# ActiveVisionLab/CrossScore

Measured on AMD Instinct MI355X. Metric: query-images/sec at 518x518, 5 ref views, bs=8; score-map MAE vs ref, higher is better.
Workload: dtype fp16

## Files before the change

crossscore_amd/_lib.py:

```python
from __future__ import annotations

import ctypes as C
import os

HERE = os.path.dirname(os.path.abspath(__file__))
LIB_PATH = os.path.join(HERE, "libcrossscore_hip.so")

CS_OK, CS_ERR_BAD_ARG, CS_ERR_UNSUPPORTED, CS_ERR_STATE, CS_ERR_HIP = range(5)
METRIC_SSIM_M1_1, METRIC_SSIM_0_1, METRIC_MAE, METRIC_MSE = range(4)
PNG_GRAY16, PNG_RGB8 = 0, 1
PNG_DYNAMIC, PNG_ADAPTIVE_FILTER = 1, 2
(PNGDEC_OK, PNGDEC_BAD_CRC, PNGDEC_BAD_ADLER, PNGDEC_BAD_ZLIB_HEADER, PNGDEC_BAD_BLOCK_TYPE, PNGDEC_BAD_STORED_LEN, PNGDEC_BAD_CODE, PNGDEC_BAD_SYMBOL,
 PNGDEC_BAD_DISTANCE, PNGDEC_STREAM_SHORT, PNGDEC_STREAM_LONG, PNGDEC_BAD_FILTER, PNGDEC_INPUT_EXHAUSTED, PNGDEC_HEADER_MISMATCH,
 PNGDEC_BAD_FRAMING) = range(15)
JPEG_GRAY, JPEG_444, JPEG_422, JPEG_420 = range(4)
(JPGDEC_OK, JPGDEC_BAD_FRAMING, JPGDEC_HEADER_MISMATCH, JPGDEC_BAD_TABLE, JPGDEC_BAD_CODE, JPGDEC_BAD_SYMBOL, JPGDEC_INPUT_EXHAUSTED,
 JPGDEC_BAD_RESTART) = range(8)
JPGDEC_BAD_SCAN = 8
JPEG_PROGRESSIVE = 1
GTMAP_SSIM, GTMAP_MAE = 0, 1

DTYPE_F32, DTYPE_F16, DTYPE_BF16 = 0, 1, 2
(EPI_BIAS_F16, EPI_BIAS_GELU_F16, EPI_BIAS_RELU_F16, EPI_BIAS_LEAKY_F16, EPI_RESID_F32, EPI_PATCH_F32, EPI_HEAD_SCORE,
 EPI_LN_F16, EPI_LN_GELU_F16, EPI_RESID_F32_LN) = range(10)
# ... 41 lines not shown
    "cs_finalize": (_i, [_vp]),
    "cs_forward": (_i, [_vp, _vp, _vp, _i, _i, _i, _i, _vp, _vp, _i, _vp, _vp]),
    "cs_encode_references": (_i, [_vp, _vp, _i, _i, _i, _vp, _vp]),
    "cs_forward_cached": (_i, [_vp, _vp, _vp, _i, _i, _i, _i, _vp, _vp, _i, _vp, _vp]),
    "cs_forward_u8": (_i, [_vp, _vp, _vp, _i, _i, _i, _i, _fp, _fp, _vp, _vp, _i, _vp, _vp]),
    "cs_encode_references_u8": (_i, [_vp, _vp, _i, _i, _i, _fp, _fp, _vp, _vp]),
    "cs_forward_cached_u8": (_i, [_vp, _vp, _vp, _i, _i, _i, _i, _fp, _fp, _vp, _vp, _i, _vp, _vp]),
    "cs_u8_input_supported": (_i, [_vp, _vp, _i, _i]),
    "cs_op_token_descriptors": (_i, [_vp, _i, _i, _i, _i, _vp, _vp]),
    "cs_op_descriptor_centre": (_i, [_vp, _i, _i, _vp, _vp]),
    "cs_op_descriptor_unit": (_i, [_vp, _i, _i, _vp, _vp, _vp]),
    "cs_op_select_references": (_i, [_vp, _i, _vp, _i, _i, _vp, _i, _vp, _vp, _vp]),
    "cs_op_gather_tokens": (_i, [_vp, _i, _i, _i, _vp, _i, _i, _vp, _vp]),
    "cs_forward_select": (_i, [_vp, _vp, _vp, _vp, _vp, _i, _vp, _i, _i, _i, _i, _vp, _vp, _i, _vp, _vp, _vp, _vp]),
    "cs_forward_select_u8": (_i, [_vp, _vp, _vp, _vp, _vp, _i, _vp, _i, _i, _i, _i, _fp, _fp, _vp, _vp, _i, _vp, _vp, _vp, _vp]),
    "cs_op_group_descriptors": (_i, [_vp, _i, _i, _vp, _i, _vp, _vp, _vp]),
    "cs_op_select_references_grouped": (_i, [_vp, _i, _vp, _vp, _vp, _vp, _i, _i, _i, _vp, _i, _vp, _vp, _vp]),
    "cs_op_gather_tokens_ex": (_i, [_vp, _i, _i, _i, _vp, _i, _i, _vp, _vp, _i]),
    "cs_forward_select_grouped": (_i, [_vp, _vp, _vp, _vp, _vp, _i, _vp, _i, _vp, _i, _vp, _i, _i, _i, _i, _vp, _vp, _i, _vp, _vp, _vp, _vp]),
    "cs_forward_select_grouped_u8": (_i, [_vp, _vp, _vp, _vp, _vp, _i, _vp, _i, _vp, _i, _vp, _i, _i, _i, _i, _fp, _fp, _vp, _vp, _i, _vp, _vp,
                                          _vp, _vp]),
    "cs_workspace_bytes": (_sz, [_vp, _i, _i, _i, _i]),
    "cs_nonfinite_count": (_i, [_vp, C.POINTER(C.c_longlong)]),
    "cs_forward_stats": (_i, [_vp, C.POINTER(C.c_int), C.POINTER(C.c_double), C.c_char_p, _sz]),
    "cs_debug_set_op_operand_dtype": (_i, [_i]),
    "cs_debug_capture": (_i, [_vp, _i]),
    "cs_debug_read": (_i, [_vp, C.c_char_p, _vp, _sz, C.POINTER(C.c_int), C.POINTER(C.c_int), C.POINTER(C.c_int64), _vp]),
    "cs_profile_enable": (_i, [_vp, _i]),
    "cs_profile_read": (_i, [_vp, _i, C.POINTER(C.c_double), C.POINTER(C.c_int), C.POINTER(C.c_double)]),
    "cs_profile_read_bytes": (_i, [_vp, _i, C.POINTER(C.c_double)]),
    "cs_op_gemm": (_i, [_vp, _i, _vp, _i, _i, _i, _i, _vp, _vp, _i, _vp, _i, _i, _vp, _i, _i, _i, _i, _f,
                        _vp, _vp, _i, _vp, _i, _vp, _f, _vp]),
    "cs_op_head_score": (_i, [_vp, _i, _vp, _i, _i, _i, _vp, _vp, _i, _i, _i, _i, _f, _vp, _vp, _vp, _vp]),
    "cs_op_attention": (_i, [_vp, _vp, _vp, _vp, _i, _i, _i, _i, _ll, _ll, _ll, _ll, _i, _i, _i, _i, _i, _f, _vp, _vp]),
    "cs_op_attention_weights": (_i, [_vp, _vp, _i, _i, _ll, _ll, _i, _i, _i, _i, _i, _f, _vp, _i, _vp, _vp]),
    "cs_op_reference_use": (_i, [_vp, _vp, _i, _i, _ll, _ll, _i, _i, _i, _i, _i, _i, _f, _vp, _vp, _vp, _vp, _vp, _vp]),
    "cs_request_reference_use": (_i, [_vp, _vp, _vp, _vp, _vp]),
    "cs_op_layernorm": (_i, [_vp, _i, _i, _vp, _vp, _f, _vp, _vp, _vp]),
    "cs_op_ln_finalize": (_i, [_vp, _i, _i, _i, _i, _f, _vp, _vp]),
    "cs_op_silu_mul": (_i, [_vp, _i, _i, _i, _vp]),
    "cs_op_im2col": (_i, [_vp, _vp, _i, _i, _i, _i, _i, _vp]),
    "cs_op_patch_embed": (_i, [_vp, _vp, _vp, _vp, _i, _i, _i, _i, _i, _i, _vp, _vp]),
    "cs_op_patch_embed_fused": (_i, [_vp, _vp, _vp, _vp, _i, _i, _i, _i, _i, _vp, _vp]),
    "cs_op_patch_embed_fused_u8": (_i, [_vp, _i, _i, _i, _i, _i, _i, _i, _i, _i, _i, _fp, _fp, _vp, _vp, _vp, _i, _i, _vp, _vp]),
    "cs_debug_patch_fused_enable": (None, [_i]),
    "cs_set_lanes": (_i, [_vp, _i]),
    "cs_redraw_lane_streams": (_i, [_vp]),
    "cs_debug_stream_probe_log": (None, [_i]),
    "cs_op_pos_bicubic": (_i, [_vp, _i, _i, _i, _i, _vp, _vp]),
    "cs_op_pos_bicubic_ex": (_i, [_vp, _i, _i, _i, _i, _i, _vp, _vp]),
    "cs_op_pe_bilinear": (_i, [_vp, _i, _i, _i, _i, _i, _vp, _vp]),
    "cs_op_pe_interp": (_i, [_vp, _i, _i, _i, _i, _i, _i, _vp, _vp]),
    "cs_op_score_to_gray16": (_i, [_vp, C.c_longlong, _i, _vp, _vp]),
    "cs_op_score_to_rgb": (_i, [_vp, C.c_longlong, C.c_float, C.c_float, _vp, _vp, _vp]),
    "cs_png_bound": (_sz, [_i, _i, _i]),
    "cs_png_workspace_bytes": (_sz, [_i, _i, _i, _i]),
    "cs_op_png_encode": (_i, [_vp, _i, _i, _i, _i, _ll, _vp, _sz, _vp, _vp, _vp]),
    "cs_op_png_encode_ex": (_i, [_vp, _i, _i, _i, _i, _ll, _vp, _sz, _vp, _vp, _vp, _i]),
    "cs_png_probe": (_i, [_vp, _sz, _vp, _vp, _i]),
    "cs_png_decode_workspace_bytes": (_sz, [_i, _i, _i, _i, _sz]),
    "cs_op_png_decode": (_i, [_vp, _vp, _vp, _vp, _vp, _sz, _i, _i, _i, _i, _vp, _ll, _vp, _vp, _vp]),
    "cs_jpeg_probe": (_i, [_vp, _sz, _vp]),
    "cs_jpeg_decode_workspace_bytes": (_sz, [_i, _i, _i, _sz]),
    "cs_op_jpeg_decode": (_i, [_vp, _vp, _vp, _sz, _i, _i, _i, _vp, _ll, _vp, _vp, _vp]),
    "cs_jpeg_probe_ex": (_i, [_vp, _sz, _i, _vp, _vp]),
    "cs_jpeg_decode_workspace_bytes_ex": (_sz, [_i, _i, _i, _sz, _i]),
    "cs_op_jpeg_decode_ex": (_i, [_vp, _vp, _vp, _sz, _i, _i, _i, _vp, _ll, _vp, _vp, _i, _vp]),
    "cs_debug_jpeg_scan_levels": (None, [_i]),
    "cs_op_denorm_to_rgb8": (_i, [_vp, _i, _i, _i, _fp, _fp, _vp, _vp]),
    "cs_op_metric_map_u16": (_i, [_vp, _i, _i, _i, _i, _i, _i, _i, _i, _i, _i, _i, _vp, _vp, _vp]),
    "cs_op_gt_metric_map_u8": (_i, [_vp, _vp, _i, _i, _i, _ll, _i, _vp, _i, _vp]),
    "cs_op_metric_map_sums_u16": (_i, [_vp, _vp, _i, _i, _i, _i, _ll, _vp, _vp]),
    "cs_op_gt_metric_sums_u8": (_i, [_vp, _vp, _i, _i, _i, _ll, _vp, _vp]),
    "cs_score_gt_workspace_bytes": (_sz, [_i, _i, _i]),
    "cs_op_score_gt_stats": (_i, [_vp, _vp, _i, _i, _i, _vp, _vp, _vp]),
    "cs_op_preprocess_u8": (_i, [_vp, _i, _i, _i, _i, _i, _i, _i, _i, _i, C.POINTER(C.c_float), C.POINTER(C.c_float), _vp, _vp, _vp]),
    "cs_op_pack_f16": (_i, [_vp, _i, _i, _vp, _i, _vp, _vp, _vp]),
    "cs_op_streams_overlap": (_i, [_vp, _vp, _vp]),
    "cs_op_ln_fold_consts": (_i, [_vp, _i, _vp, _vp, _vp, _i, _i, _vp, _vp, _vp]),
    "cs_gemm_column_tiles": (_i, [_i]),
    "cs_debug_gemm256_enable": (None, [_i]),
    "cs_debug_gemm256_kmin": (None, [_i]),
    "cs_debug_gemm_grid": (None, [_i]),
    "cs_debug_panel_impl": (None, [_i]),
    "cs_panel_supported": (_i, [_i, _i]),
    "cs_panel_image_bytes": (_sz, [_i]),
    "cs_op_panel_pack": (_i, [_vp, _vp, _vp, _vp, _vp, _vp, _vp, _vp]),
    "cs_op_linear_layernorm": (_i, [_vp, _vp, _vp, _vp, _vp, _vp, _f, _vp, _vp, _i, _i, _vp]),
    "cs_op_linear_layernorm_linear": (_i, [_vp, _vp, _vp, _vp, _vp, _vp, _f, _vp, _vp, _vp, _vp, _i, _i, _vp, _i, _i, _vp]),
    "cs_debug_rowln_enable": (None, [_i]),
    "cs_op_encoder_panel": (_i, [_vp, _vp, _vp, _vp, _vp, _vp, _vp, _i, _f, _vp]),
}

_lib = None


class CrossScoreHipError(RuntimeError):
    pass


def load() -> C.CDLL:
    global _lib
    if _lib is not None:
        return _lib
    if not os.path.exists(LIB_PATH):
        raise CrossScoreHipError(
            f"{LIB_PATH} is missing: build it with `python -m crossscore_amd.build` (hipcc --offload-arch=gfx950). "
            "The CrossScore hot path has no CPU/eager fallback.")
    lib = C.CDLL(LIB_PATH)
    for name, (res, args) in SYMBOLS.items():
        fn = getattr(lib, name)
        fn.restype = res
        fn.argtypes = args
    _lib = lib
    return lib


def last_error() -> str:
    return load().cs_last_error().decode("utf-8", "replace")


def check(rc: int) -> None:
    if rc == CS_OK:
        return
    msg = last_error()
    if rc in (CS_ERR_BAD_ARG,):
        raise ValueError(msg)
    if rc == CS_ERR_UNSUPPORTED:
        raise NotImplementedError(msg)
    raise CrossScoreHipError(msg)
```

crossscore_amd/csrc/attention.hip:

```cpp
#include "cs_common.h"
#include <atomic>
#include <math.h>
#include <type_traits>

#ifdef CS_ATTN_STAMP
__device__ unsigned long long g_attn_dbg[64 * 4 * 8];
#define CS_TS(k) do { __builtin_amdgcn_sched_barrier(0); const unsigned long long now_ = __builtin_amdgcn_s_memtime(); \
    ph[k] += now_ - tlast; tlast = now_; __builtin_amdgcn_sched_barrier(0); } while (0)
#else
#define CS_TS(k) do { } while (0)
#endif

namespace {

template <int DH>
struct AttnCfg {
  static constexpr bool T16 = DH == 48 || DH == 64;
  static constexpr int KS = DH / 16;
  static constexpr int DT = (DH + 31) / 32;
  static constexpr int KS2 = (DH + 31) / 32;
  static constexpr int DT16 = DH / 16;
  static constexpr int CH = DH / 8;
  static constexpr int KROW = T16 ? 160 : DH * 2 + 16;
  static constexpr int VROW = T16 ? (DH == 64 ? 160 : 96) : (DH <= 16) ? 64 : (DH <= 96 ? 192 : (DH <= 128 ? 320 : 448));
  static_assert(T16 ? (VROW >= DH * 2 && (VROW / 4) % 16 == 8 && KROW >= KS2 * 64 && (KROW / 16) % 4 == 2)
                    : (VROW >= DT * 64 && (VROW / 4) % 32 == 16), "K / V row pitch");
  static constexpr int KTILE = 64 * KROW;
  static constexpr int VTILE = 64 * VROW;
  static constexpr int STAGE = KTILE + VTILE;
  static constexpr int NIT = (64 * CH + 255) / 256;
};

template <int DH, bool BF>
__global__ __launch_bounds__(256, DH > 128 ? 1 : (AttnCfg<DH>::T16 ? 3 : 2)) void cs_attn_kernel(CsAttnParams p) {
  using Cfg = AttnCfg<DH>;
  constexpr int KS = Cfg::KS, DT = Cfg::DT, CH = Cfg::CH, NIT = Cfg::NIT;
  extern __shared__ __attribute__((aligned(16))) char smem[];
  const int tid = threadIdx.x;
  const int lane = tid & 63;
  const int wv = __builtin_amdgcn_readfirstlane(tid >> 6);
  const int r = lane & 31;
  const int hh = lane >> 5;
  const int QB = (p.Lq + 127) / 128;
  const int xcd = blockIdx.x & 7, jj = blockIdx.x >> 3;
  const int gi = jj / QB, qb = jj - gi * QB;
  const int grp = gi * 8 + xcd;
  if (grp >= p.heads * p.nbatch) return;
  const int head = grp % p.heads;
  const int bat = grp / p.heads;
  const int q0 = qb * 128 + wv * 32;

  const h16_t* Qb = p.Q + (size_t)bat * p.q_bs + head * DH;
  const h16_t* Kb = p.K + (size_t)bat * p.k_bs + head * DH;
  const h16_t* Vb = p.V + (size_t)bat * p.v_bs + head * DH;

  constexpr bool kFullLast = (64 * CH) % 256 == 0;
  int skey[NIT], sch[NIT];
#pragma unroll
  for (int it = 0; it < NIT; ++it) {
    const int c = tid + it * 256;
    skey[it] = c / CH;
    sch[it] = c - skey[it] * CH;
  }
  uint4 kreg[NIT], vreg[NIT];
#pragma unroll
  for (int it = 0; it < NIT; ++it) { kreg[it] = make_uint4(0, 0, 0, 0); vreg[it] = make_uint4(0, 0, 0, 0); }
  unsigned kgo[NIT], vgo[NIT];
#pragma unroll
  for (int it = 0; it < NIT; ++it) {
    kgo[it] = ((unsigned)skey[it] * (unsigned)p.ldk + (unsigned)sch[it] * 8u) * 2u;
    vgo[it] = ((unsigned)skey[it] * (unsigned)p.ldv + (unsigned)sch[it] * 8u) * 2u;
  }
  const unsigned k_bytes = (unsigned)(((size_t)(p.Lk - 1) * p.ldk + DH) * 2), v_bytes = (unsigned)(((size_t)(p.Lk - 1) * p.ldv + DH) * 2);
#define CS_ATTN_LOAD_TILE(T)                                                                       \
  {                                                                                                \
    const unsigned ks_ = (unsigned)(T) * 64u * (unsigned)p.ldk * 2u, vs_ = (unsigned)(T) * 64u * (unsigned)p.ldv * 2u; \
    const __amdgpu_buffer_rsrc_t k_rs = __builtin_amdgcn_make_buffer_rsrc(                         \
        const_cast<char*>(reinterpret_cast<const char*>(Kb)) + ks_, 0, (int)(k_bytes - ks_), 0x00020000); \
    const __amdgpu_buffer_rsrc_t v_rs = __builtin_amdgcn_make_buffer_rsrc(                         \
        const_cast<char*>(reinterpret_cast<const char*>(Vb)) + vs_, 0, (int)(v_bytes - vs_), 0x00020000); \
    _Pragma("unroll") for (int it = 0; it < NIT; ++it) {                                           \
      if (kFullLast || it + 1 < NIT || tid + it * 256 < 64 * CH) {                                 \
        kreg[it] = __builtin_bit_cast(uint4, __builtin_amdgcn_raw_buffer_load_b128(k_rs, kgo[it], 0, 0)); \
        vreg[it] = __builtin_bit_cast(uint4, __builtin_amdgcn_raw_buffer_load_b128(v_rs, vgo[it], 0, 0)); \
      }                                                                                            \
    }                                                                                              \
  }
#define CS_ATTN_WRITE_TILE(BUF)                                                                    \
  _Pragma("unroll") for (int it = 0; it < NIT; ++it) {                                             \
    if (kFullLast || it + 1 < NIT || tid + it * 256 < 64 * CH) {                                   \
      char* kb_ = smem + (BUF) * Cfg::STAGE;                                                       \
      *reinterpret_cast<uint4*>(kb_ + skey[it] * Cfg::KROW + sch[it] * 16) = kreg[it];             \
      *reinterpret_cast<uint4*>(kb_ + Cfg::KTILE + skey[it] * Cfg::VROW + sch[it] * 16) = vreg[it]; \
    }                                                                                              \
  }

  if constexpr (Cfg::T16) {
    constexpr int KS2 = Cfg::KS2, DT16 = Cfg::DT16;
    const int li = lane & 15, g = lane >> 4;
    const int nqt = __builtin_amdgcn_readfirstlane(q0 >= p.Lq ? 0 : (q0 + 16 >= p.Lq ? 1 : 2));
    if constexpr (DH == 48) {
      const int zrow = (tid >> 1) & 63;
      *reinterpret_cast<uint4*>(smem + (tid >> 7) * Cfg::STAGE + zrow * Cfg::KROW + 96 + 16 * (tid & 1)) = make_uint4(0, 0, 0, 0);
    }
    h16x8_t qf[2][KS2];
#pragma unroll
    for (int qt = 0; qt < 2; ++qt) {
      int qr = q0 + 16 * qt + li;
      qr = qr < p.Lq ? qr : p.Lq - 1;
      const h16_t* qp = Qb + (size_t)qr * p.ldq + 8 * g;
#pragma unroll
      for (int s = 0; s < KS2; ++s) {
#pragma unroll
        for (int j = 0; j < 8; ++j) qf[qt][s][j] = (_Float16)0.f;
        if (32 * s + 32 <= DH || 32 * s + 8 * g < DH) qf[qt][s] = *reinterpret_cast<const h16x8_t*>(qp + 32 * s);
      }
    }
    {
      const float sc = p.scale_log2e;
      if (sc != 1.0f) {
#pragma unroll
        for (int qt = 0; qt < 2; ++qt)
#pragma unroll
          for (int s = 0; s < KS2; ++s)
#pragma unroll
            for (int j = 0; j < 8; ++j) {
              const _Float16 e = qf[qt][s][j];
              qf[qt][s][j] = __builtin_bit_cast(_Float16, f2o<BF>(o2f<BF>(__builtin_bit_cast(h16_t, e)) * sc));
            }
      }
    }
    f32x4_t ot[2][DT16];
#pragma unroll
    for (int qt = 0; qt < 2; ++qt)
#pragma unroll
      for (int d = 0; d < DT16; ++d)
#pragma unroll
        for (int e = 0; e < 4; ++e) ot[qt][d][e] = 0.f;
    constexpr float kTau = 8.0f;
    float m_run[2] = {0.f, 0.f};
    float l_run[2] = {0.f, 0.f};
    f32x4_t negm[2];
#pragma unroll
    for (int qt = 0; qt < 2; ++qt)
#pragma unroll
      for (int e = 0; e < 4; ++e) negm[qt][e] = 0.f;

    const int koff = li * Cfg::KROW + g * 16;
    const int voff = (4 * g + (li >> 2)) * Cfg::VROW + (li & 3) * 8;

    const int nt = (p.Lk + 63) / 64;
    CS_ATTN_LOAD_TILE(0)
    CS_ATTN_WRITE_TILE(0)
    __syncthreads();
#ifdef CS_ATTN_STAMP
    unsigned long long ph[5] = {0, 0, 0, 0, 0};
    const unsigned long long tbegin = __builtin_amdgcn_s_memtime(), rbegin = __builtin_amdgcn_s_memrealtime();
    unsigned long long tlast = tbegin;
#endif
    auto tile = [&](auto full_c, const int t, const int nkt) __attribute__((always_inline)) {
      constexpr bool FULL = decltype(full_c)::value;
      const char* kb = smem + (t & 1) * Cfg::STAGE;
      const char* vb = kb + Cfg::KTILE;
      f32x4_t st[2][4];
      h16x8_t pf[2][2];
      float tm[2] = {-INFINITY, -INFINITY};
#pragma unroll
      for (int kt = 0; kt < 4; ++kt) {
        if (FULL || kt < nkt) {
          if (!FULL) __builtin_amdgcn_sched_barrier(0);
#pragma unroll
          for (int s = 0; s < KS2; ++s) {
            const h16x8_t kf = *reinterpret_cast<const h16x8_t*>(kb + koff + kt * 16 * Cfg::KROW + s * 64);
#pragma unroll
            for (int qt = 0; qt < 2; ++qt)
              if (FULL || qt < nqt) st[qt][kt] = mfma_16x16x32<BF>(kf, qf[qt][s], s == 0 ? negm[qt] : st[qt][kt]);
          }
#pragma unroll
          for (int qt = 0; qt < 2; ++qt)
            if (FULL || qt < nqt) {
              if (!FULL) {
                const int key = t * 64 + kt * 16 + 4 * g;
#pragma unroll
                for (int j = 0; j < 4; ++j)
                  if (key + j >= p.Lk) st[qt][kt][j] = -INFINITY;
              }
#pragma unroll
              for (int j = 0; j < 4; ++j) tm[qt] = fmaxf(tm[qt], st[qt][kt][j]);
            }
        }
      }
      CS_TS(0);
      if (t == 0 || __builtin_amdgcn_ballot_w64(fmaxf(tm[0], tm[1]) > kTau) != 0) {
#pragma unroll
        for (int qt = 0; qt < 2; ++qt)
          if (FULL || qt < nqt) {
            float rm = fmaxf(tm[qt], __shfl_xor(tm[qt], 16, 64));
            rm = fmaxf(rm, __shfl_xor(rm, 32, 64));
            const float delta = t == 0 ? rm : fmaxf(rm, 0.f);
            const float alpha = t == 0 ? 1.0f : __builtin_amdgcn_exp2f(-delta);
            m_run[qt] += delta;
#pragma unroll
            for (int e = 0; e < 4; ++e) negm[qt][e] = -m_run[qt];
            asm volatile("" : "+v"(negm[qt]));
#pragma unroll
            for (int kt = 0; kt < 4; ++kt)
              if (FULL || kt < nkt)
#pragma unroll
                for (int j = 0; j < 4; ++j) st[qt][kt][j] -= delta;
            l_run[qt] *= alpha;
#pragma unroll
            for (int d = 0; d < DT16; ++d)
#pragma unroll
              for (int e = 0; e < 4; ++e) ot[qt][d][e] *= alpha;
          }
      }
      if (!FULL) __builtin_amdgcn_sched_barrier(0);
#pragma unroll
      for (int qt = 0; qt < 2; ++qt)
        if (FULL || qt < nqt) {
          float ps0 = 0.f, ps1 = 0.f;
#pragma unroll
          for (int kt = 0; kt < 4; ++kt) {
            if (FULL || kt < nkt) {
#pragma unroll
              for (int j = 0; j < 4; j += 2) {
                const float pa = __builtin_amdgcn_exp2f(st[qt][kt][j]);
                const float pb = __builtin_amdgcn_exp2f(st[qt][kt][j + 1]);
                ps0 += pa;
                ps1 += pb;
                pf[qt][kt >> 1][4 * (kt & 1) + j] = __builtin_bit_cast(_Float16, f2o<BF>(pa));
                pf[qt][kt >> 1][4 * (kt & 1) + j + 1] = __builtin_bit_cast(_Float16, f2o<BF>(pb));
              }
            } else {
#pragma unroll
              for (int j = 0; j < 4; ++j) pf[qt][kt >> 1][4 * (kt & 1) + j] = (_Float16)0.f;
            }
          }
          l_run[qt] += ps0 + ps1;
        }
      CS_TS(1);
      if (!FULL) __builtin_amdgcn_sched_barrier(0);
#pragma unroll
      for (int s = 0; s < 2; ++s)
        if (FULL || 2 * s < nkt) {
          const char* vrow = vb + voff + 32 * s * Cfg::VROW;
#pragma unroll
          for (int d = 0; d < DT16; ++d) {
            short4_t lo = __builtin_amdgcn_ds_read_tr16_b64_v4i16(
                (__attribute__((address_space(3))) short4_t*)(vrow + d * 32));
            short4_t hi = __builtin_amdgcn_ds_read_tr16_b64_v4i16(
                (__attribute__((address_space(3))) short4_t*)(vrow + 16 * Cfg::VROW + d * 32));
            const short8_t vf8 = __builtin_shufflevector(lo, hi, 0, 1, 2, 3, 4, 5, 6, 7);
#pragma unroll
            for (int qt = 0; qt < 2; ++qt)
              if (FULL || qt < nqt) ot[qt][d] = mfma_16x16x32<BF>(__builtin_bit_cast(h16x8_t, vf8), pf[qt][s], ot[qt][d]);
          }
        }
      CS_TS(2);
    };
    auto run = [&](auto full_c, const int t0, const int t1) __attribute__((always_inline)) {
      for (int t = t0; t < t1; ++t) {
        if (t + 1 < nt) { CS_ATTN_LOAD_TILE(t + 1) }
        if (decltype(full_c)::value || nqt > 0) {
          const int left = p.Lk - t * 64;
          tile(full_c, t, left >= 64 ? 4 : (left + 15) >> 4);
        }
        if (t + 1 < nt) { CS_ATTN_WRITE_TILE((t + 1) & 1) }
        CS_TS(3);
        __syncthreads();
        CS_TS(4);
      }
    };
    const int ntf = nqt == 2 ? ((p.Lk & 63) ? nt - 1 : nt) : 0;
    run(std::true_type{}, 0, ntf);
    run(std::false_type{}, ntf, nt);
#ifdef CS_ATTN_STAMP
    if (blockIdx.x % 50 == 0 && blockIdx.x / 50 < 64 && lane == 0) {
      unsigned long long* d = g_attn_dbg + (blockIdx.x / 50 * 4 + wv) * 8;
      for (int k = 0; k < 5; ++k) d[k] = ph[k];
      d[5] = rbegin;
      d[6] = __builtin_amdgcn_s_memtime() - tbegin;
      d[7] = __builtin_amdgcn_s_memrealtime() - rbegin;
    }
#endif

    const int le = __builtin_amdgcn_mbcnt_hi(~0u, __builtin_amdgcn_mbcnt_lo(~0u, 0u));
    const int lie = le & 15, ge = le >> 4;
#pragma unroll
    for (int qt = 0; qt < 2; ++qt) {
      float l_tot = l_run[qt] + __shfl_xor(l_run[qt], 16, 64);
      l_tot += __shfl_xor(l_tot, 32, 64);
      const float inv = 1.0f / l_tot;
      const int q = q0 + 16 * qt + lie;
      if (q < p.Lq) {
        h16_t* op = p.O + (size_t)bat * p.o_bs + (size_t)q * p.ldo + head * DH + 4 * ge;
#pragma unroll
        for (int d = 0; d < DT16; ++d) {
          uint2 o;
          o.x = pack_o16x2<BF>(ot[qt][d][0] * inv, ot[qt][d][1] * inv);
          o.y = pack_o16x2<BF>(ot[qt][d][2] * inv, ot[qt][d][3] * inv);
          *reinterpret_cast<uint2*>(op + 16 * d) = o;
        }
        if (p.lse && ge == 0) p.lse[((size_t)bat * p.heads + head) * p.Lq + q] = m_run[qt] + log2f(l_tot);
      }
    }
  } else
  {
  h16x8_t qf[KS];
  {
    int qr = q0 + r;
    qr = qr < p.Lq ? qr : p.Lq - 1;
    const h16_t* qp = Qb + (size_t)qr * p.ldq + 8 * hh;
#pragma unroll
    for (int s = 0; s < KS; ++s) qf[s] = *reinterpret_cast<const h16x8_t*>(qp + 16 * s);
  }

  f32x16_t ot[DT];
#pragma unroll
  for (int d = 0; d < DT; ++d)
#pragma unroll
    for (int e = 0; e < 16; ++e) ot[d][e] = 0.f;
  constexpr float kTau = 8.0f;
  float m_run = 0.f;
  float l_run = 0.f;
  f32x16_t negm;
#pragma unroll
  for (int e = 0; e < 16; ++e) negm[e] = 0.f;
  {
    const float sc = p.scale_log2e;
    if (sc != 1.0f) {
#pragma unroll
      for (int s = 0; s < KS; ++s)
#pragma unroll
        for (int j = 0; j < 8; ++j) {
          const _Float16 e = qf[s][j];
          qf[s][j] = __builtin_bit_cast(_Float16, f2o<BF>(o2f<BF>(__builtin_bit_cast(h16_t, e)) * sc));
        }
    }
  }

  const int koff = r * Cfg::KROW + hh * 16;
  const int li = lane & 15, lg = (lane >> 4) & 1;
  const int voff = (4 * hh + (li >> 2)) * Cfg::VROW + (16 * lg + 4 * (li & 3)) * 2;

  const int nt = (p.Lk + 63) / 64;
  CS_ATTN_LOAD_TILE(0)
  CS_ATTN_WRITE_TILE(0)
  __syncthreads();
#ifdef CS_ATTN_STAMP
  unsigned long long ph[5] = {0, 0, 0, 0, 0};
  const unsigned long long tbegin = __builtin_amdgcn_s_memtime(), rbegin = __builtin_amdgcn_s_memrealtime();
  unsigned long long tlast = tbegin;
// ... 68 lines not shown
          for (int j = 0; j < 8; j += 2) {
            const float pa = __builtin_amdgcn_exp2f(st[k2][8 * s2 + j]);
            const float pb = __builtin_amdgcn_exp2f(st[k2][8 * s2 + j + 1]);
            ps0 += pa;
            ps1 += pb;
            pf[k2][s2][j] = __builtin_bit_cast(_Float16, f2o<BF>(pa));
            pf[k2][s2][j + 1] = __builtin_bit_cast(_Float16, f2o<BF>(pb));
          }
        }
    };
    scores();
    const float tmax = row_max();
    CS_TS(0);
    if (t == 0 || __builtin_amdgcn_ballot_w64(tmax > kTau) != 0) move_reference(t == 0 ? tmax : fmaxf(tmax, 0.f), t == 0);
    exp_pack();
    l_run += ps0 + ps1;
    CS_TS(1);

#pragma unroll
    for (int k2 = 0; k2 < 2; ++k2)
#pragma unroll
      for (int s2 = 0; s2 < 2; ++s2) {
        if (k2 == 1 && !two) continue;
        const char* vrow = vb + voff + (k2 * 32 + 16 * s2) * Cfg::VROW;
#pragma unroll
        for (int d = 0; d < DT; ++d) {
          short4_t lo = __builtin_amdgcn_ds_read_tr16_b64_v4i16(
              (__attribute__((address_space(3))) short4_t*)(vrow + d * 64));
          short4_t hi = __builtin_amdgcn_ds_read_tr16_b64_v4i16(
              (__attribute__((address_space(3))) short4_t*)(vrow + 8 * Cfg::VROW + d * 64));
          short8_t vf8 = __builtin_shufflevector(lo, hi, 0, 1, 2, 3, 4, 5, 6, 7);
          ot[d] = mfma_32x32x16<BF>(__builtin_bit_cast(h16x8_t, vf8), pf[k2][s2], ot[d]);
        }
      }

    CS_TS(2);
  };
  auto run = [&](auto last_c, const int t0, const int t1) __attribute__((always_inline)) {
    for (int t = t0; t < t1; ++t) {
      if (t + 1 < nt) { CS_ATTN_LOAD_TILE(t + 1) }
      if (live_w) tile(last_c, t);
      if (t + 1 < nt) { CS_ATTN_WRITE_TILE((t + 1) & 1) }
      CS_TS(3);
      __syncthreads();
      CS_TS(4);
    }
  };
  run(std::false_type{}, 0, nt - 1);
  run(std::true_type{}, nt - 1, nt);
#ifdef CS_ATTN_STAMP
  if (blockIdx.x % 50 == 0 && blockIdx.x / 50 < 64 && lane == 0) {
    unsigned long long* d = g_attn_dbg + (blockIdx.x / 50 * 4 + wv) * 8;
    for (int k = 0; k < 5; ++k) d[k] = ph[k];
    d[5] = rbegin;
    d[6] = __builtin_amdgcn_s_memtime() - tbegin;
    d[7] = __builtin_amdgcn_s_memrealtime() - rbegin;
  }
#endif

  const float l_tot = l_run + __shfl_xor(l_run, 32, 64);
  const float inv = 1.0f / l_tot;
  const int q = q0 + r;
  if (q < p.Lq) {
    h16_t* op = p.O + (size_t)bat * p.o_bs + (size_t)q * p.ldo + head * DH;
#pragma unroll
    for (int d = 0; d < DT; ++d)
#pragma unroll
      for (int g4 = 0; g4 < 4; ++g4) {
        const int dd = d * 32 + 8 * g4 + 4 * hh;
        if (dd < DH) {
          const float v0 = ot[d][4 * g4 + 0] * inv, v1 = ot[d][4 * g4 + 1] * inv, v2 = ot[d][4 * g4 + 2] * inv, v3 = ot[d][4 * g4 + 3] * inv;
          uint2 o;
          o.x = pack_o16x2<BF>(v0, v1);
          o.y = pack_o16x2<BF>(v2, v3);
          *reinterpret_cast<uint2*>(op + dd) = o;
        }
      }
    if (p.lse && hh == 0) p.lse[((size_t)bat * p.heads + head) * p.Lq + q] = m_run + log2f(l_tot);
  }
  }
}

template <int DH, bool BF>
hipError_t launch(CsAttnParams p, int batch, hipStream_t stream) {
  p.nbatch = batch;
  const int groups = p.heads * batch;
  dim3 grid(((groups + 7) / 8) * 8 * ((p.Lq + 127) / 128));
  const int lds = 2 * AttnCfg<DH>::STAGE + 64;
  if (lds > 48 * 1024) {
    static std::atomic<bool> attr_done[16];
    int dev = 0;
    if (hipGetDevice(&dev) != hipSuccess || dev < 0 || dev >= 16) return hipErrorInvalidDevice;
    if (!attr_done[dev]) {
      hipError_t e = hipFuncSetAttribute(reinterpret_cast<const void*>(cs_attn_kernel<DH, BF>), hipFuncAttributeMaxDynamicSharedMemorySize, lds);
      if (e != hipSuccess) return e;
      attr_done[dev] = true;
    }
  }
  hipLaunchKernelGGL((cs_attn_kernel<DH, BF>), grid, dim3(256), lds, stream, p);
  return hipGetLastError();
}

}

#ifdef CS_ATTN_STAMP
extern "C" int cs_attn_debug_read(unsigned long long* dst) { return (int)hipMemcpyFromSymbol(dst, HIP_SYMBOL(g_attn_dbg), sizeof(g_attn_dbg)); }
#endif

extern "C" const char* cs_attn_check(const CsAttnParams* p, int dh, int batch) {
  if (dh != 16 && dh != 48 && dh != 64 && dh != 96 && dh != 128 && dh != 192) return "attention: head dim must be 16, 48, 64, 96, 128 or 192";
  if (p->Lq <= 0 || p->Lk <= 0 || p->heads <= 0 || batch <= 0) return "attention: empty shape";
  if ((long long)batch * p->heads * ((p->Lq + 127) / 128) > (1ll << 30)) return "attention: grid too large";
  if (p->ldq % 8 || p->ldk % 8 || p->ldv % 8 || p->ldo % 4) return "attention: row strides must keep 16-byte rows";
  if (p->q_bs % 8 || p->k_bs % 8 || p->v_bs % 8 || p->o_bs % 4) return "attention: batch strides must keep 16-byte rows";
  if (!p->Q || !p->K || !p->V || !p->O) return "attention: null operand";
  if ((long long)p->Lk * p->ldk >= (1ll << 30) || (long long)p->Lk * p->ldv >= (1ll << 30)) return "attention: Lk * row stride must stay below 2^30 elements (32-bit tile offsets)";
  return nullptr;
}

extern "C" hipError_t cs_attn_launch(const CsAttnParams* p, int dh, int batch, hipStream_t stream) {
  switch (dh) {
    case 16: return p->bf16 ? launch<16, true>(*p, batch, stream) : launch<16, false>(*p, batch, stream);
    case 48: return p->bf16 ? launch<48, true>(*p, batch, stream) : launch<48, false>(*p, batch, stream);
    case 64: return p->bf16 ? launch<64, true>(*p, batch, stream) : launch<64, false>(*p, batch, stream);
    case 96: return p->bf16 ? launch<96, true>(*p, batch, stream) : launch<96, false>(*p, batch, stream);
    case 128: return p->bf16 ? launch<128, true>(*p, batch, stream) : launch<128, false>(*p, batch, stream);
    case 192: return p->bf16 ? launch<192, true>(*p, batch, stream) : launch<192, false>(*p, batch, stream);
  }
  return hipErrorInvalidValue;
}
```

include/crossscore_hip.h:

```cpp
#ifndef CROSSSCORE_HIP_H
#define CROSSSCORE_HIP_H

#include <stddef.h>
#include <stdint.h>

#ifdef __cplusplus
extern "C" {
#endif

typedef struct cs_model* cs_handle;
typedef void* cs_stream;

enum {
  CS_OK = 0,
  CS_ERR_BAD_ARG = 1,
  CS_ERR_UNSUPPORTED = 2,
  CS_ERR_STATE = 3,
  CS_ERR_HIP = 4
};

typedef struct cs_config {
  int hidden;
  int enc_layers;
  int enc_heads;
// ... 148 lines not shown
  CS_PNGDEC_BAD_ZLIB_HEADER = 3,
  CS_PNGDEC_BAD_BLOCK_TYPE = 4,
  CS_PNGDEC_BAD_STORED_LEN = 5,
  CS_PNGDEC_BAD_CODE = 6,
  CS_PNGDEC_BAD_SYMBOL = 7,
  CS_PNGDEC_BAD_DISTANCE = 8,
  CS_PNGDEC_STREAM_SHORT = 9,
  CS_PNGDEC_STREAM_LONG = 10,
  CS_PNGDEC_BAD_FILTER = 11,
  CS_PNGDEC_INPUT_EXHAUSTED = 12,
  CS_PNGDEC_HEADER_MISMATCH = 13,
  CS_PNGDEC_BAD_FRAMING = 14
};
int cs_png_probe(const uint8_t* file, size_t n, cs_png_info* info, cs_png_span* spans, int max_spans);
size_t cs_png_decode_workspace_bytes(int kind, int I, int H, int W, size_t total_file_bytes);
int cs_op_png_decode(const uint8_t* files, const uint64_t* file_offsets, const uint32_t* file_lengths, const cs_png_span* spans,
                     const uint32_t* span_offsets, size_t total_file_bytes, int I, int kind, int H, int W, void* pixels, long long image_stride_bytes,
                     uint32_t* status, void* workspace, cs_stream stream);
enum { CS_JPEG_GRAY = 0, CS_JPEG_444 = 1, CS_JPEG_422 = 2, CS_JPEG_420 = 3 };
typedef struct cs_jpeg_info {
  int width, height, components;
  int sampling;
  int restart_interval;
  unsigned long long entropy_offset;
} cs_jpeg_info;
enum {
  CS_JPGDEC_OK = 0,
  CS_JPGDEC_BAD_FRAMING = 1,
  CS_JPGDEC_HEADER_MISMATCH = 2,
  CS_JPGDEC_BAD_TABLE = 3,
  CS_JPGDEC_BAD_CODE = 4,
  CS_JPGDEC_BAD_SYMBOL = 5,
  CS_JPGDEC_INPUT_EXHAUSTED = 6,
  CS_JPGDEC_BAD_RESTART = 7
};
int cs_jpeg_probe(const uint8_t* file, size_t n, cs_jpeg_info* info);
size_t cs_jpeg_decode_workspace_bytes(int I, int H, int W, size_t total_file_bytes);
int cs_op_jpeg_decode(const uint8_t* files, const uint64_t* file_offsets, const uint32_t* file_lengths, size_t total_file_bytes, int I, int H,
                      int W, void* pixels, long long image_stride_bytes, uint32_t* status, void* workspace, cs_stream stream);
#define CS_JPEG_PROGRESSIVE 1
#define CS_JPGDEC_BAD_SCAN 8
typedef struct cs_jpeg_scan_info {
  int process;
  int scans;
  unsigned long long entropy_offset;
} cs_jpeg_scan_info;
int cs_jpeg_probe_ex(const uint8_t* file, size_t n, int flags, cs_jpeg_info* info, cs_jpeg_scan_info* scans);
size_t cs_jpeg_decode_workspace_bytes_ex(int I, int H, int W, size_t total_file_bytes, int flags);
int cs_op_jpeg_decode_ex(const uint8_t* files, const uint64_t* file_offsets, const uint32_t* file_lengths, size_t total_file_bytes, int I, int H,
                         int W, void* pixels, long long image_stride_bytes, uint32_t* status, void* workspace, int flags, cs_stream stream);
void cs_debug_jpeg_scan_levels(int on);
int cs_op_denorm_to_rgb8(const float* chw, int I, int H, int W, const float* mean3, const float* std3, uint8_t* out, cs_stream stream);
enum { CS_METRIC_SSIM_M1_1 = 0, CS_METRIC_SSIM_0_1 = 1, CS_METRIC_MAE = 2, CS_METRIC_MSE = 3 };
int cs_op_metric_map_u16(const uint16_t* maps, int B, int in_h, int in_w, int in_row_elems, int mode, int rs_h, int rs_w, int crop_y, int crop_x,
                         int out_h, int out_w, float* out, float* scratch, cs_stream stream);
enum { CS_GTMAP_SSIM = 0, CS_GTMAP_MAE = 1 };
int cs_op_gt_metric_map_u8(const uint8_t* render, const uint8_t* gt, int B, int H, int W, long long image_stride_bytes, int kind,
                           uint16_t* out, int out_row_elems, cs_stream stream);
int cs_op_metric_map_sums_u16(const uint16_t* ssim, const uint16_t* mae, int B, int H, int W, int row_elems, long long image_stride_elems,
                              uint64_t* sums, cs_stream stream);
int cs_op_gt_metric_sums_u8(const uint8_t* render, const uint8_t* gt, int B, int H, int W, long long image_stride_bytes, uint64_t* sums,
                            cs_stream stream);
size_t cs_score_gt_workspace_bytes(int B, int H, int W);
int cs_op_score_gt_stats(const float* score, const float* gt, int B, int H, int W, double* stats, void* scratch, cs_stream stream);
int cs_op_pos_bicubic(const float* pos, int G, int C, int gh, int gw, float* out, cs_stream stream);
int cs_op_pos_bicubic_ex(const float* pos, int G, int C, int gh, int gw, int legacy, float* out, cs_stream stream);
int cs_op_pe_bilinear(const float* pe, int ph, int pw, int C, int gh, int gw, float* out, cs_stream stream);
int cs_op_pe_interp(const float* pe, int ph, int pw, int C, int gh, int gw, int mode, float* out, cs_stream stream);
int cs_op_streams_overlap(cs_stream a, cs_stream b, int* overlap);
int cs_op_pack_f16(const float* w, int rows, int K, uint16_t* out, int ldo, const float* row_scale, const float* col_scale,
                    cs_stream stream);
int cs_op_ln_fold_consts(const uint16_t* w_packed, int ldp, const float* w, const float* beta, const float* bias, int N, int K,
                         float* s_out, float* c_out, cs_stream stream);
void cs_debug_panel_impl(int impl);
int cs_panel_supported(int hidden, int mlp_ratio);
size_t cs_panel_image_bytes(int with_outproj);
int cs_op_panel_pack(const float* wo, const float* ls1, const float* w1, const float* g2, const float* w2, const float* ls2,
                     uint16_t* img, cs_stream stream);
int cs_op_encoder_panel(float* x, const uint16_t* attn_o, const uint16_t* img, const float* bo, const float* b1, const float* b2,
                        uint16_t* u_out, int M, float eps, cs_stream stream);
void cs_debug_gemm256_enable(int on);
void cs_debug_gemm256_kmin(int k);
void cs_debug_gemm_grid(int blocks);
int cs_op_linear_layernorm(const uint16_t* A, const uint16_t* W, const float* bias, const float* resid, const float* gamma, const float* beta,
                           float eps, float* out_f32, uint16_t* out_f16, int M, int C, cs_stream stream);
int cs_op_linear_layernorm_linear(const uint16_t* A, const uint16_t* W, const float* bias, const float* resid, const float* gamma,
                                  const float* beta, float eps, float* out_f32, uint16_t* out_f16, const uint16_t* W2, const float* bias2,
                                  int n2, int act2, uint16_t* out2, int M, int C, cs_stream stream);
void cs_debug_rowln_enable(int on);
int cs_gemm_column_tiles(int N);

#ifdef __cplusplus
}
#endif
#endif
```

Measured before the change: 1422.

## Stage K/V tiles via buffer-to-LDS DMA with triple buffering for head dim 64

For head dimension 64, the attention kernel now loads K and V tiles straight from global memory into LDS using buffer_load_lds. It uses three rotating slots with a two-tile prefetch distance and a swizzled 128-byte row layout, checked for bank conflicts at compile time. V transposed reads are issued early and paired with fine-grained lgkmcnt waits so they overlap the PV MFMAs. This removes the register round-trip and the VGPR pressure of the old load/write staging. In exchange it uses 48KB of LDS, which may reduce resident blocks, and it depends on hand-counted waitcnt values. A debug occupancy query is also added.

```diff
diff --git a/crossscore_amd/_lib.py b/crossscore_amd/_lib.py
--- a/crossscore_amd/_lib.py
+++ b/crossscore_amd/_lib.py
@@ -147,6 +147,7 @@
     "cs_debug_gemm256_enable": (None, [_i]),
     "cs_debug_gemm256_kmin": (None, [_i]),
     "cs_debug_gemm_grid": (None, [_i]),
+    "cs_debug_attn_resident_blocks": (_i, [_i, _i]),
     "cs_debug_panel_impl": (None, [_i]),
     "cs_panel_supported": (_i, [_i, _i]),
     "cs_panel_image_bytes": (_sz, [_i]),
diff --git a/crossscore_amd/csrc/attention.hip b/crossscore_amd/csrc/attention.hip
--- a/crossscore_amd/csrc/attention.hip
+++ b/crossscore_amd/csrc/attention.hip
@@ -1,3 +1,4 @@
+#include "attn_stage.h"
 #include "cs_common.h"
 #include <atomic>
 #include <math.h>
@@ -29,7 +30,24 @@
   static constexpr int VTILE = 64 * VROW;
   static constexpr int STAGE = KTILE + VTILE;
   static constexpr int NIT = (64 * CH + 255) / 256;
+  static constexpr bool DMA = DH == 64;
+  static constexpr int LDS_BYTES = DMA ? attn_stage::SLOTS * attn_stage::SLOT : 2 * STAGE + 64;
 };
+#define CS_ATTN_WAIT(VM) asm volatile("s_waitcnt vmcnt(%0) lgkmcnt(0)" ::"n"(VM) : "memory")
+template <int OFF>
+__device__ __forceinline__ void attn_tr_read(unsigned addr, short4_t& w) {
+  asm volatile("ds_read_b64_tr_b16 %0, %1 offset:%2" : "=&v"(w) : "v"(addr), "n"(OFF));
+}
+template <int N>
+__device__ __forceinline__ void attn_tr_wait(short4_t& a, short4_t& b, f32x4_t& prev) {
+  static_assert(N >= 0 && N <= 15, "lgkmcnt is four bits");
+  asm volatile("s_waitcnt lgkmcnt(%3)" : "+v"(a), "+v"(b), "+v"(prev) : "n"(N));
+}
+#define CS_ATTN_V_READS(S)                                                                              \
+  _Pragma("unroll") for (int d = 0; d < 4; ++d) {                                                       \
+    attn_tr_read<attn_stage::IMAGE + 32 * S * attn_stage::ROWB>(vaddr[d], vlo[S][d]);                   \
+    attn_tr_read<attn_stage::IMAGE + (32 * S + 16) * attn_stage::ROWB>(vaddr[d], vhi[S][d]);            \
+  }
 
 template <int DH, bool BF>
 __global__ __launch_bounds__(256, DH > 128 ? 1 : (AttnCfg<DH>::T16 ? 3 : 2)) void cs_attn_kernel(CsAttnParams p) {
@@ -148,11 +166,59 @@
 
     const int koff = li * Cfg::KROW + g * 16;
     const int voff = (4 * g + (li >> 2)) * Cfg::VROW + (li & 3) * 8;
+    const int koff_x = attn_stage::k_read_byte(0, 0, lane);
+    const int voff_x = attn_stage::v_read_byte(0, 0, 0, lane);
 
     const int nt = (p.Lk + 63) / 64;
-    CS_ATTN_LOAD_TILE(0)
-    CS_ATTN_WRITE_TILE(0)
-    __syncthreads();
+    [[maybe_unused]] unsigned dko[2], dvo[2];
+    if constexpr (Cfg::DMA) {
+#pragma unroll
+      for (int e = 0; e < 2; ++e) {
+        const int key = attn_stage::piece_key(2 * wv + e, lane);
+        dko[e] = ((unsigned)key * (unsigned)p.ldk + (unsigned)attn_stage::piece_chunk(false, 2 * wv + e, lane) * 8u) * 2u;
+        dvo[e] = ((unsigned)key * (unsigned)p.ldv + (unsigned)attn_stage::piece_chunk(true, 2 * wv + e, lane) * 8u) * 2u;
+      }
+    }
+    [[maybe_unused]] auto issue = [&](const int T, const int slot) __attribute__((always_inline)) {
+      unsigned ko[2] = {dko[0], dko[1]}, vo[2] = {dvo[0], dvo[1]};
+      if (T == nt - 1 && (p.Lk & 63)) {
+        const int last = p.Lk - 1 - T * 64;
+#pragma unroll
+        for (int e = 0; e < 2; ++e) {
+          const int key = min(attn_stage::piece_key(2 * wv + e, lane), last);
+          ko[e] = ((unsigned)key * (unsigned)p.ldk + (unsigned)attn_stage::piece_chunk(false, 2 * wv + e, lane) * 8u) * 2u;
+          vo[e] = ((unsigned)key * (unsigned)p.ldv + (unsigned)attn_stage::piece_chunk(true, 2 * wv + e, lane) * 8u) * 2u;
+        }
+      }
+      const unsigned ks_ = (unsigned)T * 64u * (unsigned)p.ldk * 2u, vs_ = (unsigned)T * 64u * (unsigned)p.ldv * 2u;
+      const __amdgpu_buffer_rsrc_t k_rs = __builtin_amdgcn_make_buffer_rsrc(
+          const_cast<char*>(reinterpret_cast<const char*>(Kb)) + ks_, 0, (int)(k_bytes - ks_), 0x00020000);
+      const __amdgpu_buffer_rsrc_t v_rs = __builtin_amdgcn_make_buffer_rsrc(
+          const_cast<char*>(reinterpret_cast<const char*>(Vb)) + vs_, 0, (int)(v_bytes - vs_), 0x00020000);
+      char* dst = smem + slot * attn_stage::SLOT + 2 * wv * attn_stage::PIECE;
+#pragma unroll
+      for (int e = 0; e < 2; ++e) __builtin_amdgcn_raw_ptr_buffer_load_lds(k_rs, CS_LDS_PTR(dst + e * attn_stage::PIECE), 16, ko[e], 0, 0, 0);
+#pragma unroll
+      for (int e = 0; e < 2; ++e)
+        __builtin_amdgcn_raw_ptr_buffer_load_lds(v_rs, CS_LDS_PTR(dst + attn_stage::IMAGE + e * attn_stage::PIECE), 16, vo[e], 0, 0, 0);
+    };
+    int rslot = 0;
+    if constexpr (Cfg::DMA) {
+      issue(0, 0);
+      if (nt > 1) {
+        issue(1, 1);
+        CS_ATTN_WAIT(4);
+      } else {
+        CS_ATTN_WAIT(0);
+      }
+      __builtin_amdgcn_sched_barrier(0);
+      __builtin_amdgcn_s_barrier();
+      __builtin_amdgcn_sched_barrier(0);
+    } else {
+      CS_ATTN_LOAD_TILE(0)
+      CS_ATTN_WRITE_TILE(0)
+      __syncthreads();
+    }
 #ifdef CS_ATTN_STAMP
     unsigned long long ph[5] = {0, 0, 0, 0, 0};
     const unsigned long long tbegin = __builtin_amdgcn_s_memtime(), rbegin = __builtin_amdgcn_s_memrealtime();
@@ -160,8 +226,8 @@
 #endif
     auto tile = [&](auto full_c, const int t, const int nkt) __attribute__((always_inline)) {
       constexpr bool FULL = decltype(full_c)::value;
-      const char* kb = smem + (t & 1) * Cfg::STAGE;
-      const char* vb = kb + Cfg::KTILE;
+      const char* kb = Cfg::DMA ? smem + rslot * attn_stage::SLOT : smem + (t & 1) * Cfg::STAGE;
+      const char* vb = kb + (Cfg::DMA ? attn_stage::IMAGE : Cfg::KTILE);
       f32x4_t st[2][4];
       h16x8_t pf[2][2];
       float tm[2] = {-INFINITY, -INFINITY};
@@ -171,7 +237,8 @@
           if (!FULL) __builtin_amdgcn_sched_barrier(0);
 #pragma unroll
           for (int s = 0; s < KS2; ++s) {
-            const h16x8_t kf = *reinterpret_cast<const h16x8_t*>(kb + koff + kt * 16 * Cfg::KROW + s * 64);
+            const h16x8_t kf = *reinterpret_cast<const h16x8_t*>(Cfg::DMA ? kb + (koff_x ^ (s * 64)) + kt * 16 * attn_stage::ROWB
+                                                                          : kb + koff + kt * 16 * Cfg::KROW + s * 64);
 #pragma unroll
             for (int qt = 0; qt < 2; ++qt)
               if (FULL || qt < nqt) st[qt][kt] = mfma_16x16x32<BF>(kf, qf[qt][s], s == 0 ? negm[qt] : st[qt][kt]);
@@ -214,6 +281,14 @@
 #pragma unroll
               for (int e = 0; e < 4; ++e) ot[qt][d][e] *= alpha;
           }
+      }
+      [[maybe_unused]] short4_t vlo[2][4], vhi[2][4];
+      [[maybe_unused]] unsigned vaddr[4];
+      if constexpr (Cfg::DMA) {
+        const unsigned vbase = (unsigned)(size_t)CS_LDS_PTR(smem) + rslot * attn_stage::SLOT;
+#pragma unroll
+        for (int d = 0; d < 4; ++d) vaddr[d] = vbase + (voff_x ^ (d * 32));
+        if constexpr (FULL) { CS_ATTN_V_READS(0) }
       }
       if (!FULL) __builtin_amdgcn_sched_barrier(0);
 #pragma unroll
@@ -241,34 +316,74 @@
         }
       CS_TS(1);
       if (!FULL) __builtin_amdgcn_sched_barrier(0);
-#pragma unroll
-      for (int s = 0; s < 2; ++s)
-        if (FULL || 2 * s < nkt) {
-          const char* vrow = vb + voff + 32 * s * Cfg::VROW;
-#pragma unroll
-          for (int d = 0; d < DT16; ++d) {
-            short4_t lo = __builtin_amdgcn_ds_read_tr16_b64_v4i16(
-                (__attribute__((address_space(3))) short4_t*)(vrow + d * 32));
-            short4_t hi = __builtin_amdgcn_ds_read_tr16_b64_v4i16(
-                (__attribute__((address_space(3))) short4_t*)(vrow + 16 * Cfg::VROW + d * 32));
-            const short8_t vf8 = __builtin_shufflevector(lo, hi, 0, 1, 2, 3, 4, 5, 6, 7);
-#pragma unroll
-            for (int qt = 0; qt < 2; ++qt)
-              if (FULL || qt < nqt) ot[qt][d] = mfma_16x16x32<BF>(__builtin_bit_cast(h16x8_t, vf8), pf[qt][s], ot[qt][d]);
-          }
-        }
+      if constexpr (Cfg::DMA) {
+#define CS_ATTN_PV_D(S, D, BEHIND)                                                                                       \
+  {                                                                                                                     \
+    attn_tr_wait<BEHIND>(vlo[S][D], vhi[S][D], ot[0][(D + 3) & 3]);                                                     \
+    const short8_t vf8 = __builtin_shufflevector(vlo[S][D], vhi[S][D], 0, 1, 2, 3, 4, 5, 6, 7);                         \
+    _Pragma("unroll") for (int qt = 0; qt < 2; ++qt)                                                                    \
+      if (FULL || qt < nqt) ot[qt][D] = mfma_16x16x32<BF>(__builtin_bit_cast(h16x8_t, vf8), pf[qt][S], ot[qt][D]);      \
+  }
+#define CS_ATTN_PV(S, YOUNGER) CS_ATTN_PV_D(S, 0, YOUNGER + 6) CS_ATTN_PV_D(S, 1, YOUNGER + 4) CS_ATTN_PV_D(S, 2, YOUNGER + 2) CS_ATTN_PV_D(S, 3, YOUNGER)
+        if constexpr (FULL) {
+          CS_ATTN_V_READS(1)
+          CS_ATTN_PV(0, 8)
+          CS_ATTN_PV(1, 0)
+        } else {
+          CS_ATTN_V_READS(0)
+          CS_ATTN_PV(0, 0)
+          if (2 < nkt) {
+            CS_ATTN_V_READS(1)
+            CS_ATTN_PV(1, 0)
+          }
+        }
+#undef CS_ATTN_PV
+#undef CS_ATTN_PV_D
+      } else {
+#pragma unroll
+        for (int s = 0; s < 2; ++s)
+          if (FULL || 2 * s < nkt) {
+            const char* vrow = vb + voff + 32 * s * Cfg::VROW;
+#pragma unroll
+            for (int d = 0; d < DT16; ++d) {
+              short4_t lo = __builtin_amdgcn_ds_read_tr16_b64_v4i16(
+                  (__attribute__((address_space(3))) short4_t*)(vrow + d * 32));
+              short4_t hi = __builtin_amdgcn_ds_read_tr16_b64_v4i16(
+                  (__attribute__((address_space(3))) short4_t*)(vrow + 16 * Cfg::VROW + d * 32));
+              const short8_t vf8 = __builtin_shufflevector(lo, hi, 0, 1, 2, 3, 4, 5, 6, 7);
+#pragma unroll
+              for (int qt = 0; qt < 2; ++qt)
+                if (FULL || qt < nqt) ot[qt][d] = mfma_16x16x32<BF>(__builtin_bit_cast(h16x8_t, vf8), pf[qt][s], ot[qt][d]);
+            }
+          }
+      }
       CS_TS(2);
     };
     auto run = [&](auto full_c, const int t0, const int t1) __attribute__((always_inline)) {
       for (int t = t0; t < t1; ++t) {
-        if (t + 1 < nt) { CS_ATTN_LOAD_TILE(t + 1) }
+        if constexpr (Cfg::DMA) {
+          if (t + 2 < nt) issue(t + 2, rslot == 0 ? 2 : rslot - 1);
+        } else {
+          if (t + 1 < nt) { CS_ATTN_LOAD_TILE(t + 1) }
+        }
         if (decltype(full_c)::value || nqt > 0) {
           const int left = p.Lk - t * 64;
           tile(full_c, t, left >= 64 ? 4 : (left + 15) >> 4);
         }
-        if (t + 1 < nt) { CS_ATTN_WRITE_TILE((t + 1) & 1) }
-        CS_TS(3);
-        __syncthreads();
+        if constexpr (Cfg::DMA) {
+          __builtin_amdgcn_sched_barrier(0);
+          if (t + 2 < nt) CS_ATTN_WAIT(4);
+          else CS_ATTN_WAIT(0);
+          CS_TS(3);
+          __builtin_amdgcn_sched_barrier(0);
+          __builtin_amdgcn_s_barrier();
+          __builtin_amdgcn_sched_barrier(0);
+          rslot = rslot == 2 ? 0 : rslot + 1;
+        } else {
+          if (t + 1 < nt) { CS_ATTN_WRITE_TILE((t + 1) & 1) }
+          CS_TS(3);
+          __syncthreads();
+        }
         CS_TS(4);
       }
     };
@@ -503,11 +618,8 @@
 }
 
 template <int DH, bool BF>
-hipError_t launch(CsAttnParams p, int batch, hipStream_t stream) {
-  p.nbatch = batch;
-  const int groups = p.heads * batch;
-  dim3 grid(((groups + 7) / 8) * 8 * ((p.Lq + 127) / 128));
-  const int lds = 2 * AttnCfg<DH>::STAGE + 64;
+hipError_t allow_lds() {
+  constexpr int lds = AttnCfg<DH>::LDS_BYTES;
   if (lds > 48 * 1024) {
     static std::atomic<bool> attr_done[16];
     int dev = 0;
@@ -518,8 +630,25 @@
       attr_done[dev] = true;
     }
   }
-  hipLaunchKernelGGL((cs_attn_kernel<DH, BF>), grid, dim3(256), lds, stream, p);
+  return hipSuccess;
+}
+
+template <int DH, bool BF>
+hipError_t launch(CsAttnParams p, int batch, hipStream_t stream) {
+  p.nbatch = batch;
+  const int groups = p.heads * batch;
+  dim3 grid(((groups + 7) / 8) * 8 * ((p.Lq + 127) / 128));
+  if (hipError_t e = allow_lds<DH, BF>(); e != hipSuccess) return e;
+  hipLaunchKernelGGL((cs_attn_kernel<DH, BF>), grid, dim3(256), AttnCfg<DH>::LDS_BYTES, stream, p);
   return hipGetLastError();
+}
+
+template <int DH, bool BF>
+int resident_blocks() {
+  int n = 0;
+  if (allow_lds<DH, BF>() != hipSuccess) return -1;
+  if (hipOccupancyMaxActiveBlocksPerMultiprocessor(&n, reinterpret_cast<const void*>(cs_attn_kernel<DH, BF>), 256, AttnCfg<DH>::LDS_BYTES) != hipSuccess) return -1;
+  return n;
 }
 
 }
@@ -550,3 +679,15 @@
   }
   return hipErrorInvalidValue;
 }
+
+extern "C" int cs_debug_attn_resident_blocks(int dh, int bf16) {
+  switch (dh) {
+    case 16: return bf16 ? resident_blocks<16, true>() : resident_blocks<16, false>();
+    case 48: return bf16 ? resident_blocks<48, true>() : resident_blocks<48, false>();
+    case 64: return bf16 ? resident_blocks<64, true>() : resident_blocks<64, false>();
+    case 96: return bf16 ? resident_blocks<96, true>() : resident_blocks<96, false>();
+    case 128: return bf16 ? resident_blocks<128, true>() : resident_blocks<128, false>();
+    case 192: return bf16 ? resident_blocks<192, true>() : resident_blocks<192, false>();
+  }
+  return -1;
+}
diff --git a/crossscore_amd/csrc/attn_stage.h b/crossscore_amd/csrc/attn_stage.h
--- /dev/null
+++ b/crossscore_amd/csrc/attn_stage.h
@@ -0,0 +1,91 @@
+#pragma once
+
+namespace attn_stage {
+
+constexpr int ROWB = 128;
+constexpr int IMAGE = 64 * ROWB;
+constexpr int SLOT = 2 * IMAGE;
+constexpr int SLOTS = 3;
+constexpr int PIECE = 1024;
+constexpr int PIECES = IMAGE / PIECE;
+
+constexpr int swz(bool v, int key) { return v ? ((key >> 1) & 3) << 1 : (key >> 1) & 7; }
+constexpr int lds_byte(bool v, int key, int chunk) { return key * ROWB + ((chunk ^ swz(v, key)) << 4); }
+constexpr int piece_key(int piece, int lane) { return piece * 8 + (lane >> 3); }
+constexpr int piece_chunk(bool v, int piece, int lane) { return (lane & 7) ^ swz(v, piece_key(piece, lane)); }
+
+constexpr int k_read_byte(int kt, int s, int lane) { return lds_byte(false, 16 * kt + (lane & 15), 4 * s + (lane >> 4)); }
+constexpr int v_read_byte(int s, int h, int d, int lane) {
+  const int li = lane & 15, g = lane >> 4;
+  return lds_byte(true, 32 * s + 16 * h + 4 * g + (li >> 2), 2 * d + ((li & 3) >> 1)) + 8 * (li & 1);
+}
+
+namespace check {
+constexpr bool dma_is_bijection(bool v) {
+  bool seen[64 * 8] = {};
+  for (int p = 0; p < PIECES; ++p)
+    for (int l = 0; l < 64; ++l) {
+      const int key = piece_key(p, l), ch = piece_chunk(v, p, l);
+      if (key < 0 || key >= 64 || ch < 0 || ch >= 8 || seen[key * 8 + ch]) return false;
+      seen[key * 8 + ch] = true;
+      if (lds_byte(v, key, ch) != p * PIECE + 16 * l) return false;
+    }
+  for (int i = 0; i < 64 * 8; ++i)
+    if (!seen[i]) return false;
+  return true;
+}
+constexpr bool group_conflict_free(const int* addr, int n, int bytes) {
+  int owner[64] = {};
+  for (int i = 0; i < 64; ++i) owner[i] = -1;
+  for (int i = 0; i < n; ++i)
+    for (int b = 0; b < bytes / 4; ++b) {
+      const int bank = (addr[i] / 4 + b) & 63;
+      if (owner[bank] >= 0 && owner[bank] != addr[i] + 4 * b) return false;
+      owner[bank] = addr[i] + 4 * b;
+    }
+  return true;
+}
+constexpr int B128_GROUP[4][16] = {{0, 1, 2, 3, 12, 13, 14, 15, 20, 21, 22, 23, 24, 25, 26, 27},
+                                   {4, 5, 6, 7, 8, 9, 10, 11, 16, 17, 18, 19, 28, 29, 30, 31},
+                                   {32, 33, 34, 35, 44, 45, 46, 47, 52, 53, 54, 55, 56, 57, 58, 59},
+                                   {36, 37, 38, 39, 40, 41, 42, 43, 48, 49, 50, 51, 60, 61, 62, 63}};
+constexpr bool k_reads_conflict_free() {
+  for (int kt = 0; kt < 4; ++kt)
+    for (int s = 0; s < 2; ++s)
+      for (int grp = 0; grp < 4; ++grp) {
+        int addr[16] = {};
+        for (int i = 0; i < 16; ++i) addr[i] = k_read_byte(kt, s, B128_GROUP[grp][i]);
+        if (!group_conflict_free(addr, 16, 16)) return false;
+      }
+  return true;
+}
+constexpr bool v_reads_conflict_free() {
+  for (int s = 0; s < 2; ++s)
+    for (int h = 0; h < 2; ++h)
+      for (int d = 0; d < 4; ++d)
+        for (int grp = 0; grp < 2; ++grp) {
+          int addr[32] = {};
+          for (int i = 0; i < 32; ++i) addr[i] = v_read_byte(s, h, d, 32 * grp + i);
+          if (!group_conflict_free(addr, 32, 8)) return false;
+        }
+  return true;
+}
+constexpr bool read_steps_are_lane_independent() {
+  for (int l = 0; l < 64; ++l) {
+    for (int kt = 0; kt < 4; ++kt)
+      for (int s = 0; s < 2; ++s)
+        if (k_read_byte(kt, s, l) != (k_read_byte(0, 0, l) ^ (64 * s)) + kt * 16 * ROWB) return false;
+    for (int s = 0; s < 2; ++s)
+      for (int h = 0; h < 2; ++h)
+        for (int d = 0; d < 4; ++d)
+          if (v_read_byte(s, h, d, l) != (v_read_byte(0, 0, 0, l) ^ (32 * d)) + (32 * s + 16 * h) * ROWB) return false;
+  }
+  return true;
+}
+static_assert(dma_is_bijection(false) && dma_is_bijection(true), "LDS-DMA map: every (key, chunk) exactly once, where the reads look for it");
+static_assert(k_reads_conflict_free(), "K fragment reads: 64 distinct banks per lane group");
+static_assert(v_reads_conflict_free(), "V transposed reads: 64 distinct banks per lane group");
+static_assert(read_steps_are_lane_independent(), "read addresses: per-lane offset + compile-time step");
+}
+
+}
diff --git a/include/crossscore_hip.h b/include/crossscore_hip.h
--- a/include/crossscore_hip.h
+++ b/include/crossscore_hip.h
@@ -254,6 +254,7 @@
 void cs_debug_gemm256_enable(int on);
 void cs_debug_gemm256_kmin(int k);
 void cs_debug_gemm_grid(int blocks);
+int cs_debug_attn_resident_blocks(int dh, int bf16);
 int cs_op_linear_layernorm(const uint16_t* A, const uint16_t* W, const float* bias, const float* resid, const float* gamma, const float* beta,
                            float eps, float* out_f32, uint16_t* out_f16, int M, int C, cs_stream stream);
 int cs_op_linear_layernorm_linear(const uint16_t* A, const uint16_t* W, const float* bias, const float* resid, const float* gamma,
```

New measurement: 1430, median of 6. Within noise of the previous version (+0.6%).
